# weiguangzhao/PBNet

Measured on AMD Instinct MI355X. Metric: scenes/sec fwd+cluster (ScanNet ~150k pts/scene), higher is better.
Workload: dtype bf16; 1 GPU; configs[1]: 1 scene, 161517 pts, 146038 voxels @2cm, 1 rotated copy, full PBNet.forward (MinkUNet34C + grouping + MinkUNet14A mask + MinkUNet34C score); scenes_in_flight_per_gpu=4, scene_seeds=2 (configs[1])

## Files before the change

pbnet_amd/csrc/cluster.hip:

```cpp
#include "pbn_common.h"

#pragma clang fp contract(off)

namespace pbn {
namespace {

constexpr int TPB = 256;
constexpr unsigned long long EMPTY_KEY = ~0ULL;
constexpr int CELL_BIAS = 32768;
constexpr float CELL_CLAMP = 32764.0f;
constexpr int CELL_R = 2;
constexpr int BIG = 0x7f7f7f7f;

__constant__ float c_mean_count[18] = {3917.0f, 12056.0f, 2303.0f, 8331.0f, 3948.0f, 3166.0f, 5629.0f, 11719.0f, 1003.0f,
                                       3317.0f, 4912.0f,  10221.0f, 3889.0f, 4136.0f, 2120.0f, 945.0f,  3967.0f, 2589.0f};

__device__ __forceinline__ float sqdist(float ax, float ay, float az, float bx, float by, float bz) {
    const float dx = __fsub_rn(ax, bx), dy = __fsub_rn(ay, by), dz = __fsub_rn(az, bz);
    const float a = __fmul_rn(dx, dx), b = __fmul_rn(dy, dy), c = __fmul_rn(dz, dz);
    return __fadd_rn(__fadd_rn(a, b), c);
}

__device__ __forceinline__ int cls_of(int sem) { return min(max(sem - 2, 0), 17); }

__device__ __forceinline__ int cell_coord(float v, float inv_cell) {
    float f = floorf(v * inv_cell);
    f = fminf(fmaxf(f, -CELL_CLAMP), CELL_CLAMP);
    return (int)f;
}

__device__ __forceinline__ unsigned long long pack_key(int seg, int cx, int cy, int cz) {
    return ((unsigned long long)(unsigned)seg << 48) | ((unsigned long long)(unsigned)(cx + CELL_BIAS) << 32) |
           ((unsigned long long)(unsigned)(cy + CELL_BIAS) << 16) | (unsigned long long)(unsigned)(cz + CELL_BIAS);
}

__device__ __forceinline__ int hash_lookup(const unsigned long long* __restrict__ hkeys, unsigned hmask,
                                           unsigned long long key) {
    unsigned h = hash64(key) & hmask;
    for (unsigned probes = 0; probes <= hmask; ++probes) {
        unsigned long long k = hkeys[h];
        if (k == key) return (int)h;
        if (k == EMPTY_KEY) return -1;
        h = (h + 1) & hmask;
    }
    return -1;
}

__global__ void k_seg_offsets(const int* __restrict__ seg_len, int n_seg, int n, int capacity, int* __restrict__ seg_off,
                              int* __restrict__ status) {
    const int lane = lane_id();
    int carry = 0;
    int bad = 0;
    for (int base = 0; base < n_seg; base += 64) {
        int i = base + lane;
        int v = (i < n_seg) ? seg_len[i] : 0;
        if (v < 0) bad = 1;
        int incl = v;
#pragma unroll
        for (int o = 1; o < 64; o <<= 1) {
            int t = __shfl_up(incl, o, 64);
            if (lane >= o) incl += t;
        }
        if (i < n_seg) seg_off[i] = carry + incl - v;
        carry += __shfl(incl, 63, 64);
    }
    bad = __any(bad);
    if (lane == 0) {
        seg_off[n_seg] = carry;
        if ((capacity ? carry > n : carry != n) || bad) atomicOr(status, 1);
    }
}

struct NRef {
    int cap;
    const int* dev;
    __device__ __forceinline__ int get() const { return dev ? min(cap, *dev) : cap; }
};

__device__ __forceinline__ int find_segment(const int* __restrict__ seg_off, int n_seg, int i) {
    int lo = 0, hi = n_seg;
    while (hi - lo > 1) {
        int mid = (lo + hi) >> 1;
        if (seg_off[mid] <= i) lo = mid; else hi = mid;
    }
    return lo;
}

__global__ __launch_bounds__(TPB) void k_cell_insert(const float* __restrict__ off_xyz, const int* __restrict__ sem,
                                                    const int* __restrict__ seg_off, int n_seg, NRef n_ref, float inv_cell,
                                                    unsigned long long* __restrict__ hkeys, int* __restrict__ hcount,
                                                    unsigned hmask, int* __restrict__ slot_of_pt,
                                                    int* __restrict__ seg_of_pt, int* __restrict__ status) {
    const int n = n_ref.get();
    const int i = blockIdx.x * TPB + threadIdx.x;
    if (i >= n) return;
    const int s = sem[i];
    if (s < 2 || s > 19) atomicOr(status, 2);
    const int seg = find_segment(seg_off, n_seg, i);
    seg_of_pt[i] = seg;
    const float x = off_xyz[3 * i + 0], y = off_xyz[3 * i + 1], z = off_xyz[3 * i + 2];
    const unsigned long long key = pack_key(seg, cell_coord(x, inv_cell), cell_coord(y, inv_cell), cell_coord(z, inv_cell));
    unsigned h = hash64(key) & hmask;
    bool placed = false;
    for (unsigned probes = 0; probes <= hmask; ++probes) {
        unsigned long long prev = atomicCAS(&hkeys[h], EMPTY_KEY, key);
        if (prev == EMPTY_KEY || prev == key) { placed = true; break; }
        h = (h + 1) & hmask;
    }
    if (!placed) { atomicOr(status, 4); h = 0; }
    atomicAdd(&hcount[h], 1);
    slot_of_pt[i] = (int)h;
}

__global__ __launch_bounds__(TPB) void k_cell_scatter(const float* __restrict__ off_xyz, NRef n_ref,
                                                     const int* __restrict__ slot_of_pt, const int* __restrict__ hstart,
                                                     int* __restrict__ hcursor, const int* __restrict__ seg_of_pt,
                                                     float4* __restrict__ spt, int* __restrict__ sseg,
                                                     int* __restrict__ sslot) {
    const int n = n_ref.get();
    const int i = blockIdx.x * TPB + threadIdx.x;
    if (i >= n) return;
    const int slot = slot_of_pt[i];
    const int pos = hstart[slot] + atomicAdd(&hcursor[slot], 1);
    spt[pos] = make_float4(off_xyz[3 * i + 0], off_xyz[3 * i + 1], off_xyz[3 * i + 2], __int_as_float(i));
    sseg[pos] = seg_of_pt[i];
    sslot[pos] = slot;
}

__device__ __forceinline__ bool cell_trusted(int cx, int cy, int cz) {
    const int lim = (int)CELL_CLAMP;
    return cx > -lim && cx < lim && cy > -lim && cy < lim && cz > -lim && cz < lim;
}

template <typename F>
__device__ __forceinline__ void for_each_neighbour_cell(float x, float y, float z, int seg, float inv_cell,
                                                        const unsigned long long* __restrict__ hkeys, unsigned hmask,
                                                        const int* __restrict__ hstart, const int* __restrict__ hcount,
                                                        int first, int stride, F&& f) {
    const int cx = cell_coord(x, inv_cell), cy = cell_coord(y, inv_cell), cz = cell_coord(z, inv_cell);
    constexpr int W = 2 * CELL_R + 1;
    for (int c = first; c < W * W * W; c += stride) {
        const int dz = c / (W * W) - CELL_R, dy = (c / W) % W - CELL_R, dx = c % W - CELL_R;
        const int slot = hash_lookup(hkeys, hmask, pack_key(seg, cx + dx, cy + dy, cz + dz));
        if (slot < 0) continue;
        const int beg = hstart[slot];
        f(beg, beg + hcount[slot], slot, cell_trusted(cx + dx, cy + dy, cz + dz), (dx | dy | dz) == 0);
    }
}

constexpr int NB_Q = 8;
__device__ __forceinline__ bool group_any(bool pred) {
    const unsigned long long m = __ballot(pred);
    return ((m >> (threadIdx.x & 63 & ~(NB_Q - 1))) & ((1ULL << NB_Q) - 1ULL)) != 0ULL;
}
template <typename F>
__device__ __forceinline__ void for_each_neighbour_cell_group(float x, float y, float z, int seg, float inv_cell,
                                                              const unsigned long long* __restrict__ hkeys, unsigned hmask,
                                                              const int* __restrict__ hstart,
                                                              const int* __restrict__ hcount, int q, F&& f) {
    const int cx = cell_coord(x, inv_cell), cy = cell_coord(y, inv_cell), cz = cell_coord(z, inv_cell);
    constexpr int W = 2 * CELL_R + 1;
    const int gbase = (threadIdx.x & 63) & ~(NB_Q - 1);
    for (int r = 0; r < W * W * W; r += NB_Q) {
        const int c = r + q;
        int slot = -1, beg = 0, end = 0;
        if (c < W * W * W) {
            const int dz = c / (W * W) - CELL_R, dy = (c / W) % W - CELL_R, dx = c % W - CELL_R;
            slot = hash_lookup(hkeys, hmask, pack_key(seg, cx + dx, cy + dy, cz + dz));
            if (slot >= 0) { beg = hstart[slot]; end = beg + hcount[slot]; }
        }
#pragma unroll
        for (int k = 0; k < NB_Q; ++k) {
            const int sk = __shfl(slot, gbase + k, 64);
            if (sk < 0) continue;
            const int bk = __shfl(beg, gbase + k, 64), ek = __shfl(end, gbase + k, 64);
            const int ck = r + k;
            const int dz = ck / (W * W) - CELL_R, dy = (ck / W) % W - CELL_R, dx = ck % W - CELL_R;
            f(bk, ek, sk, cell_trusted(cx + dx, cy + dy, cz + dz), (dx | dy | dz) == 0);
        }
    }
}
__device__ __forceinline__ int group_sum(int v) {
#pragma unroll
    for (int o = 1; o < NB_Q; o <<= 1) v += __shfl_xor(v, o, 64);
    return v;
}
__device__ __forceinline__ int group_max(int v) {
#pragma unroll
    for (int o = 1; o < NB_Q; o <<= 1) v = max(v, __shfl_xor(v, o, 64));
    return v;
}
__constant__ unsigned short c_nb_ring[125] = {
    146, 73,  74,  75,  81,  82,  83,  89,  90,  91,  137, 138, 139, 145, 147, 153, 154, 155, 201, 202, 203, 209, 210, 211, 217,
    218, 219, 0,   1,   2,   3,   4,   8,   9,   10,  11,  12,  16,  17,  18,  19,  20,  24,  25,  26,  27,  28,  32,  33,  34,
    35,  36,  64,  65,  66,  67,  68,  72,  76,  80,  84,  88,  92,  96,  97,  98,  99,  100, 128, 129, 130, 131, 132, 136, 140,
    144, 148, 152, 156, 160, 161, 162, 163, 164, 192, 193, 194, 195, 196, 200, 204, 208, 212, 216, 220, 224, 225, 226, 227, 228,
    256, 257, 258, 259, 260, 264, 265, 266, 267, 268, 272, 273, 274, 275, 276, 280, 281, 282, 283, 284, 288, 289, 290, 291, 292};

__global__ __launch_bounds__(TPB) void k_count(const float4* __restrict__ spt, const int* __restrict__ sseg,
                                              const int* __restrict__ sslot, NRef n_ref, float inv_cell, float r2,
                                              const unsigned long long* __restrict__ hkeys, unsigned hmask,
                                              const int* __restrict__ hstart, const int* __restrict__ hcount, int min_pts,
                                              int need_den, int* __restrict__ den) {
    __shared__ float4 s_cand[TPB / 64][64];
    const int n = n_ref.get();
    if (n <= 0) return;
    const long long t = (long long)blockIdx.x * TPB + threadIdx.x;
    if ((t - (threadIdx.x & 63)) / NB_Q >= n) return;
    int p = (int)(t / NB_Q);
    const int q = (int)(t % NB_Q);
    const bool live = p < n;
    if (!live) p = n - 1;
    const float4 me = spt[p];
    const int seg = sseg[p];
    const int lane = threadIdx.x & 63, wave = threadIdx.x >> 6;
    const int gbase = lane & ~(NB_Q - 1);
    float4* line = s_cand[wave];
    const int cx = cell_coord(me.x, inv_cell), cy = cell_coord(me.y, inv_cell), cz = cell_coord(me.z, inv_cell);
    const bool own_trusted = cell_trusted(cx, cy, cz);
    int cnt = (own_trusted && q == 0) ? hcount[sslot[p]] : 0;
    bool gdone = !live;
    if (!need_den) gdone = gdone || group_sum(cnt) > min_pts;
    bool wdone = __all(gdone);
    constexpr int NCELL = (2 * CELL_R + 1) * (2 * CELL_R + 1) * (2 * CELL_R + 1);
    for (int r = 0; r < NCELL && !wdone; r += NB_Q) {
        const int c = r + q;
        int slot = -1, beg = 0, end = 0;
        if (c < NCELL && !gdone && !(c == 0 && own_trusted)) {
            const int o = c_nb_ring[c];
            const int dx = (o & 7) - CELL_R, dy = ((o >> 3) & 7) - CELL_R, dz = (o >> 6) - CELL_R;
            slot = hash_lookup(hkeys, hmask, pack_key(seg, cx + dx, cy + dy, cz + dz));
            if (slot >= 0) { beg = hstart[slot]; end = beg + hcount[slot]; }
        }
        const bool same = beg == __shfl(beg, q, 64) && end == __shfl(end, q, 64);
        if (__all(same)) {
#pragma unroll 1
            for (int k = 0; k < NB_Q && !wdone; ++k) {
                const int bk = __shfl(beg, k, 64), ek = __shfl(end, k, 64);
                float4 nxt = make_float4(0.f, 0.f, 0.f, 0.f);
                if (bk + lane < ek) nxt = spt[bk + lane];
                for (int cb = bk; cb < ek; cb += 64) {
                    line[lane] = nxt;
                    if (cb + 64 + lane < ek) nxt = spt[cb + 64 + lane];
                    const int m = min(64, ek - cb);
#pragma unroll
                    for (int i = 0; i < 64 / NB_Q; ++i) {
                        const int idx = q + NB_Q * i;
                        if (idx < m) {
                            const float4 v = line[idx];
                            cnt += (sqdist(me.x, me.y, me.z, v.x, v.y, v.z) <= r2) ? 1 : 0;
                        }
                    }
                    if (!need_den) {
                        gdone = gdone || group_sum(cnt) > min_pts;
                        wdone = __all(gdone);
                        if (wdone) break;
                    }
                }
            }
        } else {
#pragma unroll
            for (int k = 0; k < NB_Q; ++k) {
                const int sk = __shfl(slot, gbase + k, 64);
                if (sk < 0 || gdone) continue;
                const int bk = __shfl(beg, gbase + k, 64), ek = __shfl(end, gbase + k, 64);
                int j = bk + q;
                for (; j + NB_Q < ek; j += 2 * NB_Q) {
                    const float4 q0 = spt[j], q1 = spt[j + NB_Q];
                    cnt += (sqdist(me.x, me.y, me.z, q0.x, q0.y, q0.z) <= r2) ? 1 : 0;
                    cnt += (sqdist(me.x, me.y, me.z, q1.x, q1.y, q1.z) <= r2) ? 1 : 0;
                }
                for (; j < ek; j += NB_Q) {
                    const float4 q0 = spt[j];
                    cnt += (sqdist(me.x, me.y, me.z, q0.x, q0.y, q0.z) <= r2) ? 1 : 0;
                }
                if (!need_den) gdone = group_sum(cnt) > min_pts;
            }
            wdone = __all(gdone);
        }
    }
    cnt = group_sum(cnt);
    if (live && q == 0) den[__float_as_int(me.w)] = need_den ? cnt - 1 : min(cnt - 1, min_pts);
}

__global__ __launch_bounds__(TPB) void k_tag_hp(float4* __restrict__ spt, NRef n_ref, const int* __restrict__ den, int min_pts,
                                               int* __restrict__ parent, int* __restrict__ lab,
                                               const int* __restrict__ sslot, int* __restrict__ cell_rep) {
    const int n = n_ref.get();
    const int p = blockIdx.x * TPB + threadIdx.x;
    if (p >= n) return;
    const int i = __float_as_int(spt[p].w);
    const int hp = den[i] >= min_pts;
    spt[p].w = __int_as_float(i | (hp ? (int)0x80000000 : 0));
    parent[i] = i;
    lab[i] = -1;
    if (hp) atomicMin(&cell_rep[sslot[p]], i);
}

__device__ __forceinline__ int uf_load(int* p) { return __hip_atomic_load(p, __ATOMIC_RELAXED, __HIP_MEMORY_SCOPE_AGENT); }

__device__ __forceinline__ int uf_find(int* __restrict__ parent, int x) {
    while (true) {
        const int p = uf_load(&parent[x]);
        if (p == x) return x;
        const int gp = uf_load(&parent[p]);
        if (gp == p) return p;
        atomicMin(&parent[x], gp);
        x = gp;
    }
}

__device__ __forceinline__ int uf_union(int* __restrict__ parent, int a, int b) {
    while (true) {
        a = uf_find(parent, a);
        b = uf_find(parent, b);
        if (a == b) return a;
        if (a < b) { const int t = a; a = b; b = t; }
        const int old = atomicMin(&parent[a], b);
        if (old == a) return b;
        a = old;
    }
}

template <int PASS>
__global__ __launch_bounds__(TPB) void k_union(const float4* __restrict__ spt, const int* __restrict__ sseg, NRef n_ref,
                                              float inv_cell, float r2, const unsigned long long* __restrict__ hkeys,
                                              unsigned hmask, const int* __restrict__ hstart,
                                              const int* __restrict__ hcount, int* parent,
                                              const int* __restrict__ cell_rep, const int* __restrict__ sslot,
                                              int* __restrict__ unres) {
    constexpr int pass = PASS;
    const int n = n_ref.get();
    const long long t = (long long)blockIdx.x * TPB + threadIdx.x;
    const int p = (int)(t / NB_Q), q = (int)(t % NB_Q);
    if (p >= n) return;
    const float4 me = spt[p];
    const int wi = __float_as_int(me.w);
    if (wi >= 0) return;
    const int i = wi & 0x7fffffff;
    const int my_slot = sslot[p];
    const bool own_trusted = cell_trusted(cell_coord(me.x, inv_cell), cell_coord(me.y, inv_cell), cell_coord(me.z, inv_cell));
    if (pass == 1 && own_trusted && !unres[my_slot]) return;
    const int my_rep = cell_rep[my_slot];
    bool unresolved = false;
    int ri = (pass == 0) ? i : parent[i];
    if (pass == 0 && own_trusted) {
        if (my_rep != i) {
            if (q == 0) uf_union(parent, i, my_rep);
            return;
        }
    }
    for_each_neighbour_cell(me.x, me.y, me.z, sseg[p], inv_cell, hkeys, hmask, hstart, hcount, q, NB_Q,
                            [&](int beg, int end, int slot, bool trusted, bool same) {
        const int rep = cell_rep[slot];
        if (rep == BIG) return;
        if (trusted) {
            if (same) return;
            if (rep == ri || parent[rep] == ri) return;
            ri = uf_find(parent, ri);
            if (uf_find(parent, rep) == ri) return;
            constexpr int WIT = PASS == 0 ? 8 : 1;
            for (int j = beg; j < end; j += WIT) {
                float4 c[WIT];
#pragma unroll
                for (int u = 0; u < WIT; ++u) c[u] = (j + u < end) ? spt[j + u] : make_float4(0.f, 0.f, 0.f, 0.f);
#pragma unroll
                for (int u = 0; u < WIT; ++u) {
                    if (__float_as_int(c[u].w) < 0 && sqdist(me.x, me.y, me.z, c[u].x, c[u].y, c[u].z) <= r2) {
                        ri = uf_union(parent, ri, __float_as_int(c[u].w) & 0x7fffffff);
                        return;
                    }
                }
            }
            unresolved = true;
            return;
        }
        unresolved = true;
        for (int j = beg; j < end; ++j) {
            const float4 q = spt[j];
            const int wj = __float_as_int(q.w);
            const int jj = wj & 0x7fffffff;
            if (wj < 0 && jj < i && sqdist(me.x, me.y, me.z, q.x, q.y, q.z) <= r2) {
                if (parent[jj] != ri) ri = uf_union(parent, ri, jj);
            }
        }
    });
    if (pass == 0 && own_trusted && unresolved) unres[my_slot] = 1;
}

__global__ __launch_bounds__(TPB) void k_compress(const float4* __restrict__ spt, NRef n_ref, int* parent) {
    const int n = n_ref.get();
    const int p = blockIdx.x * TPB + threadIdx.x;
    if (p >= n) return;
    const int wi = __float_as_int(spt[p].w);
    if (wi >= 0) return;
    const int i = wi & 0x7fffffff;
    const int r = uf_find(parent, i);
    if (r != i) atomicMin(&parent[i], r);
}

__global__ __launch_bounds__(TPB) void k_flatten(const float4* __restrict__ spt, NRef n_ref, int* __restrict__ parent,
                                                const int* __restrict__ sem, int general, int* __restrict__ semseed,
                                                int* __restrict__ lab) {
    const int n = n_ref.get();
    const int p = blockIdx.x * TPB + threadIdx.x;
    if (p >= n) return;
    const int wi = __float_as_int(spt[p].w);
    if (wi >= 0) return;
    const int i = wi & 0x7fffffff;
    const int r = uf_find(parent, i);
    lab[i] = r;
    if (general) atomicMin(&semseed[(size_t)cls_of(sem[i]) * n + r], i);
}

__global__ __launch_bounds__(TPB) void k_hp_seed_general(const float4* __restrict__ spt, NRef n_ref, const int* __restrict__ sem,
                                                        const int* __restrict__ semseed, int* __restrict__ lab) {
    const int n = n_ref.get();
    const int p = blockIdx.x * TPB + threadIdx.x;
    if (p >= n) return;
    const int wi = __float_as_int(spt[p].w);
    if (wi >= 0) return;
    const int i = wi & 0x7fffffff;
    lab[i] = semseed[(size_t)cls_of(sem[i]) * n + lab[i]];
}

__global__ __launch_bounds__(TPB) void k_border(const float4* __restrict__ spt, const int* __restrict__ sseg, NRef n_ref,
                                               float inv_cell, float r2, const unsigned long long* __restrict__ hkeys,
                                               unsigned hmask, const int* __restrict__ hstart,
                                               const int* __restrict__ hcount, const int* __restrict__ sem, int general,
                                               const int* __restrict__ semseed, const int* __restrict__ root,
                                               int* __restrict__ lab, const int* __restrict__ cell_rep) {
    const int n = n_ref.get();
    const long long t = (long long)blockIdx.x * TPB + threadIdx.x;
    if (n <= 0 || (t - (threadIdx.x & 63)) / NB_Q >= n) return;
    int p = (int)(t / NB_Q);
    const int q = (int)(t % NB_Q);
    const bool live = p < n;
    if (!live) p = n - 1;
    const float4 me = spt[p];
    const int wi = __float_as_int(me.w);
    if (wi < 0) return;
    const int i = wi;
    const int my_cls = cls_of(sem[i]);
    int best = -1;
    auto seed_of = [&](int hp_index) {
        int s = root[hp_index];
        if (general) {
            s = semseed[(size_t)my_cls * n + s];
            if (s == BIG) s = -1;
        }
        return s;
    };
    for_each_neighbour_cell_group(me.x, me.y, me.z, sseg[p], inv_cell, hkeys, hmask, hstart, hcount, q,
                                  [&](int beg, int end, int slot, bool trusted, bool same) {
        const int rep = cell_rep[slot];
        if (rep == BIG) return;
        if (trusted) {
            const int s = seed_of(rep);
            if (s <= best) return;
            if (same) { best = s; return; }
            for (int j0 = beg; j0 < end; j0 += NB_Q) {
                const int j = j0 + q;
                bool hit = false;
                if (j < end) {
                    const float4 c = spt[j];
                    hit = __float_as_int(c.w) < 0 && sqdist(me.x, me.y, me.z, c.x, c.y, c.z) <= r2;
                }
                if (group_any(hit)) { best = s; return; }
            }
            return;
        }
        for (int j0 = beg; j0 < end; j0 += NB_Q) {
            const int j = j0 + q;
            int cand = -1;
            if (j < end) {
                const float4 c = spt[j];
                const int wj = __float_as_int(c.w);
                if (wj < 0 && sqdist(me.x, me.y, me.z, c.x, c.y, c.z) <= r2) cand = seed_of(wj & 0x7fffffff);
            }
            best = max(best, group_max(cand));
        }
    });
    best = group_max(best);
    if (live && q == 0) lab[i] = best;
}

__global__ __launch_bounds__(TPB) void k_copy_i32(const int* __restrict__ src, int* __restrict__ dst, NRef n_ref) {
    const int n = n_ref.get();
    const int i = blockIdx.x * TPB + threadIdx.x;
    if (i < n) dst[i] = src[i];
}

__global__ __launch_bounds__(TPB) void k_sizes(const int* __restrict__ lab, NRef n_ref, int* __restrict__ size) {
    const int n = n_ref.get();
    const int i = blockIdx.x * TPB + threadIdx.x;
    int s = (i < n) ? lab[i] : -1;
    unsigned long long todo = __ballot(s >= 0);
    while (todo) {
        const int leader = __ffsll((long long)todo) - 1;
        const int ls = __shfl(s, leader, 64);
        const unsigned long long same = __ballot(s == ls);
        if (lane_id() == leader) atomicAdd(&size[ls], __popcll(same));
        todo &= ~same;
    }
}

__global__ __launch_bounds__(TPB) void k_keep(const int* __restrict__ lab, const int* __restrict__ size,
                                             const int* __restrict__ sem, NRef n_ref, float para_f, int* __restrict__ keep) {
    const int n = n_ref.get();
    const int i = blockIdx.x * TPB + threadIdx.x;
    if (i >= n) return;
    int k = 0;
    if (lab[i] == i) {
        const int cs = cls_of(sem[i]);
        const float thr = __fmul_rn(c_mean_count[cs], para_f);
        k = ((float)size[i] < thr) ? 0 : 1;
    }
    keep[i] = k;
}

__global__ __launch_bounds__(TPB) void k_relabel(const int* __restrict__ lab, const int* __restrict__ keep,
                                                const int* __restrict__ newid, const int* __restrict__ sem,
                                                const int* __restrict__ seg_of_pt, const float* __restrict__ org_xyz,
                                                NRef n_ref, int* __restrict__ lab2, int* __restrict__ cluster_id,
                                                int* __restrict__ clt_sem, int* __restrict__ clt_seg,
                                                int* __restrict__ last_assigned, int* __restrict__ fsize,
                                                int* __restrict__ noise_flag, float4* __restrict__ cand,
                                                const int* __restrict__ size) {
    const int n = n_ref.get();
    if (n <= 0) return;
    int i = blockIdx.x * TPB + threadIdx.x;
    if (i - (int)(threadIdx.x & 63) >= n) return;
    const bool live = i < n;
    if (!live) i = n - 1;
    const int s = lab[i];
    const int id = (s >= 0 && keep[s]) ? newid[s] : -1;
    if (live) {
        lab2[i] = id;
        cluster_id[i] = id;
        noise_flag[i] = id < 0;
    }
    if (keep[i]) {
        clt_sem[newid[i]] = sem[i];
        clt_seg[newid[i]] = seg_of_pt[i];
        fsize[newid[i]] = size[i];
    }
    {
        const int seg = seg_of_pt[i];
        const int cand_i = (id >= 0) ? i : -1;
        const int seg0 = __shfl(seg, 0, 64);
        if (__all(seg == seg0)) {
            int m = cand_i;
#pragma unroll
            for (int o = 32; o > 0; o >>= 1) m = max(m, __shfl_xor(m, o, 64));
            if (lane_id() == 0 && m >= 0) atomicMax(&last_assigned[seg0], m);
        } else if (cand_i >= 0) {
            atomicMax(&last_assigned[seg], cand_i);
        }
    }
    if (live)
        cand[i] = make_float4(org_xyz[3 * i + 0], org_xyz[3 * i + 1], org_xyz[3 * i + 2],
                              __int_as_float(id >= 0 ? ((seg_of_pt[i] << 8) | sem[i]) : -1));
}

__global__ void k_cluster_num(const int* __restrict__ newid, const int* __restrict__ seg_off, int n_seg, NRef n_ref,
                              const int* __restrict__ total, int* __restrict__ cluster_num,
                              const int* __restrict__ status, int* __restrict__ n_clusters) {
    const int n = n_ref.get();
    const int b = blockIdx.x * blockDim.x + threadIdx.x;
    if (b == 0) *n_clusters = (*status != 0) ? -1 : *total;
    if (b >= n_seg) return;
    const int lo = seg_off[b], hi = seg_off[b + 1];
    const int a = (lo < n) ? newid[lo] : *total;
    const int e = (hi < n) ? newid[hi] : *total;
    cluster_num[b] = e - a;
}

__global__ __launch_bounds__(TPB) void k_compact_noise(const int* __restrict__ noise_flag, const int* __restrict__ pos,
                                                      NRef n_ref, int* __restrict__ noise_list) {
    const int n = n_ref.get();
    const int i = blockIdx.x * TPB + threadIdx.x;
    if (i < n && noise_flag[i]) noise_list[pos[i]] = i;
}

__global__ __launch_bounds__(TPB) void k_noise_nn(const int* __restrict__ noise_list, const int* __restrict__ n_noise,
                                                 const float4* __restrict__ cand, const int* __restrict__ sem,
                                                 const int* __restrict__ seg_of_pt, const int* __restrict__ seg_off,
                                                 const int* __restrict__ lab2, const int* __restrict__ last_assigned,
                                                 int* __restrict__ cluster_id, int* __restrict__ fsize) {
    const int lane = lane_id();
    const int w = (int)(((long long)blockIdx.x * TPB + threadIdx.x) >> 6);
    if (w >= *n_noise) return;
    const int i = noise_list[w];
    const int seg = seg_of_pt[i];
    const int beg = seg_off[seg], end = seg_off[seg + 1];
    const float4 me = cand[i];
    const int key = (seg << 8) | sem[i];
    float best = __builtin_inff();
    int bi = -1;
    for (int j = beg + lane; j < end; j += 64) {
        const float4 q = cand[j];
        if (__float_as_int(q.w) == key) {
            const float d = sqdist(me.x, me.y, me.z, q.x, q.y, q.z);
            if (d <= best) { best = d; bi = j; }
        }
    }
#pragma unroll
    for (int o = 32; o > 0; o >>= 1) {
        const float ob = __shfl_xor(best, o, 64);
        const int oi = __shfl_xor(bi, o, 64);
        if (oi >= 0 && (bi < 0 || ob < best || (ob == best && oi > bi))) { best = ob; bi = oi; }
    }
    if (lane != 0) return;
    if (bi < 0) bi = last_assigned[seg];
    const int id = (bi >= 0) ? lab2[bi] : -1;
    cluster_id[i] = id;
    if (id >= 0) atomicAdd(&fsize[id], 1);
}

__device__ __forceinline__ float exact_quotient(float d, float n, float y) {
    const float q0 = __fmul_rn(d, y);
    const float r = __fmaf_rn(-q0, n, d);
    return __fmaf_rn(r, y, q0);
}

constexpr int CTR_TPB = 64;
constexpr int CTR_SUB = 4;
constexpr int CTR_CHUNK = CTR_TPB * CTR_SUB;
__global__ __launch_bounds__(CTR_TPB) void k_centers(const int* __restrict__ cluster_id, const float* __restrict__ off_xyz,
                                                    const int* __restrict__ clt_seg, const int* __restrict__ seg_off,
                                                    const int* __restrict__ n_clusters_total,
                                                    const int* __restrict__ member_start, int* __restrict__ member_idx,
                                                    float* __restrict__ centers) {
    __shared__ __attribute__((aligned(16))) float s_xyz[3][CTR_CHUNK + 32];
    __shared__ __attribute__((aligned(16))) float s_rcp[CTR_CHUNK + 32];
    const int lane = threadIdx.x;
    const int C = *n_clusters_total;
    for (int c = blockIdx.x; c < C; c += gridDim.x) {
        const int seg = clt_seg[c];
        const int beg = seg_off[seg], end = seg_off[seg + 1];
        int wpos = member_start[c];
        int N = 0;
        float m = 0.f;
        bool hit_n[CTR_SUB];
        float nx[CTR_SUB], ny[CTR_SUB], nz[CTR_SUB];
#pragma unroll
        for (int j = 0; j < CTR_SUB; ++j) {
            const int i = beg + j * CTR_TPB + lane;
            hit_n[j] = (i < end) && (cluster_id[i] == c);
            nx[j] = ny[j] = nz[j] = 0.f;
            if (hit_n[j]) { nx[j] = off_xyz[3 * i + 0]; ny[j] = off_xyz[3 * i + 1]; nz[j] = off_xyz[3 * i + 2]; }
        }
        for (int base = beg; base < end; base += CTR_CHUNK) {
            bool hit[CTR_SUB];
            float px[CTR_SUB], py[CTR_SUB], pz[CTR_SUB];
#pragma unroll
            for (int j = 0; j < CTR_SUB; ++j) { hit[j] = hit_n[j]; px[j] = nx[j]; py[j] = ny[j]; pz[j] = nz[j]; }
#pragma unroll
            for (int j = 0; j < CTR_SUB; ++j) {
                const int i = base + CTR_CHUNK + j * CTR_TPB + lane;
                hit_n[j] = (i < end) && (cluster_id[i] == c);
                if (hit_n[j]) { nx[j] = off_xyz[3 * i + 0]; ny[j] = off_xyz[3 * i + 1]; nz[j] = off_xyz[3 * i + 2]; }
            }
            int cnt = 0;
            bool ok = true;
#pragma unroll
            for (int j = 0; j < CTR_SUB; ++j) {
                const unsigned long long mask = __ballot(hit[j]);
                const int rank = cnt + __popcll(mask & ((1ULL << lane) - 1ULL));
                cnt += __popcll(mask);
                const float ax = fabsf(px[j]), ay = fabsf(py[j]), az = fabsf(pz[j]);
                ok = ok && (!hit[j] || ((ax == 0.f || (ax >= 1e-20f && ax <= 1e20f)) && (ay == 0.f || (ay >= 1e-20f && ay <= 1e20f)) &&
                                        (az == 0.f || (az >= 1e-20f && az <= 1e20f))));
                if (hit[j]) {
                    s_xyz[0][rank] = px[j]; s_xyz[1][rank] = py[j]; s_xyz[2][rank] = pz[j];
                    if (member_idx) member_idx[wpos + rank] = base + j * CTR_TPB + lane;
                }
            }
            if (cnt == 0) continue;
            const bool fast = __all(ok);
#pragma unroll
            for (int j = 0; j < CTR_SUB; ++j)
                if (j * CTR_TPB < cnt) s_rcp[j * CTR_TPB + lane] = __fdiv_rn(1.0f, (float)(N + 1 + j * CTR_TPB + lane));
            wpos += cnt;
            __syncthreads();
            if (lane < 3) {
                const float* v = s_xyz[lane];
                if (fast) {
                    float4 va[4], ya[4], vb[4], yb[4];
                    auto load16 = [&](float4 (&vv)[4], float4 (&yy)[4], int k) {
#pragma unroll
                        for (int q = 0; q < 4; ++q) {
                            vv[q] = *reinterpret_cast<const float4*>(v + k + 4 * q);
                            yy[q] = *reinterpret_cast<const float4*>(s_rcp + k + 4 * q);
                        }
                    };
                    auto chain16 = [&](const float4 (&vv)[4], const float4 (&yy)[4], int k) {
                        const float n0 = (float)(N + k + 1);
                        const int left = cnt - k;
                        if (left >= 16) {
#pragma unroll
                            for (int q = 0; q < 4; ++q) {
                                m = __fadd_rn(m, exact_quotient(__fsub_rn(vv[q].x, m), n0 + (float)(4 * q + 0), yy[q].x));
                                m = __fadd_rn(m, exact_quotient(__fsub_rn(vv[q].y, m), n0 + (float)(4 * q + 1), yy[q].y));
                                m = __fadd_rn(m, exact_quotient(__fsub_rn(vv[q].z, m), n0 + (float)(4 * q + 2), yy[q].z));
                                m = __fadd_rn(m, exact_quotient(__fsub_rn(vv[q].w, m), n0 + (float)(4 * q + 3), yy[q].w));
                            }
                        } else {
                            for (int j = 0; j < left; ++j)
                                m = __fadd_rn(m, exact_quotient(__fsub_rn(v[k + j], m), n0 + (float)j, s_rcp[k + j]));
                        }
                    };
                    load16(va, ya, 0);
                    for (int k = 0; k < cnt; k += 32) {
                        load16(vb, yb, k + 16);
                        chain16(va, ya, k);
                        if (k + 16 < cnt) {
                            load16(va, ya, k + 32);
                            chain16(vb, yb, k + 16);
                        }
                    }
                } else {
                    for (int k = 0; k < cnt; ++k) m = __fadd_rn(m, __fdiv_rn(__fsub_rn(v[k], m), (float)(N + k + 1)));
                }
            }
            N += cnt;
            __syncthreads();
        }
        if (lane < 3) centers[3 * c + lane] = m;
    }
}

__global__ void k_member_tail(int* __restrict__ member_start, const int* __restrict__ total_assigned, int n,
                              const int* __restrict__ n_clusters) {
    if (threadIdx.x == 0 && blockIdx.x == 0) member_start[n] = *total_assigned;
    (void)n_clusters;
}

struct Workspace {
    int *seg_off, *seg_of_pt, *slot_of_pt, *hcount, *hstart, *hcursor, *unres, *sseg, *sslot, *cell_rep, *parent, *lab, *root, *semseed, *size,
        *keep, *newid, *lab2, *clt_seg, *last_assigned, *fsize, *noise_flag, *noise_pos, *noise_list, *scan_tmp,
        *scalars, *mstart_tmp;
    unsigned long long* scan_state[4];
    unsigned long long* hkeys;
    float4 *spt, *cand;
    unsigned hcap;
    size_t zero_end, ff_end, big_end;
};

unsigned hash_capacity(int n) {
    unsigned c = 1024;
    while (c < 2u * (unsigned)n) c <<= 1;
    return c;
}

size_t carve(Carver& cv, Workspace& w, int n, int n_seg, int general) {
    const size_t N = (size_t)(n > 0 ? n : 1);
    w.hcap = hash_capacity(n);
    w.scalars = cv.take<int>(64);
    for (int j = 0; j < 4; ++j)
        w.scan_state[j] = cv.take<unsigned long long>(scan_chained_state_words((long long)(w.hcap > N ? w.hcap : N)));
    w.hcount = cv.take<int>(w.hcap);
    w.hcursor = cv.take<int>(w.hcap);
    w.unres = cv.take<int>(w.hcap);
    w.size = cv.take<int>(N);
    w.fsize = cv.take<int>(N);
    w.zero_end = cv.off;
    w.hkeys = cv.take<unsigned long long>(w.hcap);
    w.last_assigned = cv.take<int>((size_t)n_seg + 1);
    w.ff_end = cv.off;
    w.cell_rep = cv.take<int>(w.hcap);
    w.semseed = cv.take<int>(general ? 18 * N : 1);
    w.big_end = cv.off;
    w.hstart = cv.take<int>(w.hcap);
    w.spt = cv.take<float4>(N);
    w.cand = cv.take<float4>(N);
    w.seg_off = cv.take<int>((size_t)n_seg + 1);
    w.seg_of_pt = cv.take<int>(N);
    w.slot_of_pt = cv.take<int>(N);
    w.sseg = cv.take<int>(N);
    w.sslot = cv.take<int>(N);
    w.parent = cv.take<int>(N);
    w.lab = cv.take<int>(N);
    w.root = cv.take<int>(N);
    w.keep = cv.take<int>(N);
    w.newid = cv.take<int>(N);
    w.lab2 = cv.take<int>(N);
    w.clt_seg = cv.take<int>(N);
    w.noise_flag = cv.take<int>(N);
    w.noise_pos = cv.take<int>(N);
    w.noise_list = cv.take<int>(N);
    w.mstart_tmp = cv.take<int>(N + 1);
    w.scan_tmp = cv.take<int>(scan_tmp_ints((long long)(w.hcap > N ? w.hcap : N)));
    return align_up(cv.off, 256);
}

}
}

using namespace pbn;

extern "C" size_t pbn_cluster_workspace_bytes(int n_points, int n_segments, int general_sem) {
    if (n_points < 0 || n_segments < 0) return 0;
    Carver cv(nullptr, 0);
    Workspace w;
    return carve(cv, w, n_points, n_segments, general_sem);
}

extern "C" int pbn_binary_cluster(const float* off_xyz, const float* org_xyz, const int32_t* sem,
                                  const int32_t* seg_len, int n, int n_seg, float radius, int min_pts, float para_f,
                                  int nv_flag, int flags, int32_t* cluster_id, int32_t* cluster_num, int32_t* den,
                                  float* centers, int32_t* clt_sem, int32_t* n_clusters, int32_t* member_start,
                                  int32_t* member_idx, void* workspace, size_t workspace_bytes, pbn_stream_t stream_) {
    hipStream_t stream = (hipStream_t)stream_;
    const int general = flags & 1;
    const int capacity = (flags >> 1) & 1;
    const int need_den = !((flags >> 2) & 1);
    if (n < 0 || n_seg < 0 || n_seg > 65535 || !(radius > 0.0f) || !n_clusters || (n_seg > 0 && !cluster_num))
        return PBN_ERR_ARG;
    if ((member_start == nullptr) != (member_idx == nullptr)) return PBN_ERR_ARG;
    if (n > 0 && (!off_xyz || !org_xyz || !sem || !seg_len || !cluster_id || !den || !centers || !clt_sem || !workspace))
        return PBN_ERR_ARG;
    if (n == 0 || n_seg == 0) {
        if (n_seg > 0) { const int frc_ = fill_bytes(cluster_num, 0, sizeof(int) * (size_t)n_seg, stream); if (frc_ != PBN_OK) return frc_; }
        { const int frc_ = fill_bytes(n_clusters, 0, sizeof(int), stream); if (frc_ != PBN_OK) return frc_; }
        if (member_start) { const int frc_ = fill_bytes(member_start, 0, sizeof(int) * ((size_t)n + 1), stream); if (frc_ != PBN_OK) return frc_; }
        return PBN_OK;
    }
    Carver cv(workspace, workspace_bytes);
    Workspace w;
    carve(cv, w, n, n_seg, general);
    if (!cv.ok) return PBN_ERR_WORKSPACE;

    const float cell = radius * 0.5625f;
    const float inv_cell = 1.0f / cell;
    const float r2 = radius * radius;
    const unsigned hmask = w.hcap - 1;
    const int nb = cdiv(n, TPB);
    const NRef nr{n, capacity ? w.seg_off + n_seg : nullptr};
    int* status = w.scalars + 0;
    int* total_kept = w.scalars + 1;
    int* n_noise = w.scalars + 2;
    int* total_assigned = w.scalars + 3;

    {
        char* base = (char*)workspace;
        char* z0 = (char*)w.scalars;
        char* f0 = (char*)w.hkeys;
        char* b0 = (char*)w.cell_rep;
        FillRange fr[7] = {{cluster_num, sizeof(int) * (size_t)n_seg, 0}, {n_clusters, sizeof(int), 0},
                           {z0, (size_t)(base + w.zero_end - z0), 0}, {f0, (size_t)(base + w.ff_end - f0), 0xff},
                           {b0, (size_t)(base + w.big_end - b0), 0x7f}, {nullptr, 0, 0}, {nullptr, 0, 0}};
        if (capacity) {
            fr[5] = FillRange{w.keep, sizeof(int) * (size_t)n, 0};
            fr[6] = FillRange{w.noise_flag, sizeof(int) * (size_t)n, 0};
        }
        const int frc = fill_ranges(fr, 7, stream);
        if (frc != PBN_OK) return frc;
    }

    hipLaunchKernelGGL(k_seg_offsets, dim3(1), dim3(64), 0, stream, seg_len, n_seg, n, capacity, w.seg_off, status);
    hipLaunchKernelGGL(k_cell_insert, dim3(nb), dim3(TPB), 0, stream, off_xyz, sem, w.seg_off, n_seg, nr, inv_cell,
                       w.hkeys, w.hcount, hmask, w.slot_of_pt, w.seg_of_pt, status);
    int rc = scan_exclusive_i32_chained(w.hcount, w.hstart, (int)w.hcap, w.scan_state[0], nullptr, status, stream);
    if (rc != PBN_OK) return rc;
    hipLaunchKernelGGL(k_cell_scatter, dim3(nb), dim3(TPB), 0, stream, off_xyz, nr, w.slot_of_pt, w.hstart, w.hcursor,
                       w.seg_of_pt, w.spt, w.sseg, w.sslot);
    hipLaunchKernelGGL(k_count, dim3(cdiv((long long)n * NB_Q, TPB)), dim3(TPB), 0, stream, w.spt, w.sseg, w.sslot, nr, inv_cell, r2,
                       w.hkeys, hmask, w.hstart, w.hcount, min_pts, need_den, den);
    hipLaunchKernelGGL(k_tag_hp, dim3(nb), dim3(TPB), 0, stream, w.spt, nr, den, min_pts, w.parent, w.lab, w.sslot, w.cell_rep);
    const dim3 nbq(cdiv((long long)n * NB_Q, TPB));
    hipLaunchKernelGGL(k_union<0>, nbq, dim3(TPB), 0, stream, w.spt, w.sseg, nr, inv_cell, r2, w.hkeys, hmask,
                       w.hstart, w.hcount, w.parent, w.cell_rep, w.sslot, w.unres);
    hipLaunchKernelGGL(k_compress, dim3(nb), dim3(TPB), 0, stream, w.spt, nr, w.parent);
    hipLaunchKernelGGL(k_union<1>, nbq, dim3(TPB), 0, stream, w.spt, w.sseg, nr, inv_cell, r2, w.hkeys, hmask,
                       w.hstart, w.hcount, w.parent, w.cell_rep, w.sslot, w.unres);
    hipLaunchKernelGGL(k_flatten, dim3(nb), dim3(TPB), 0, stream, w.spt, nr, w.parent, sem, general, w.semseed, w.lab);
    hipLaunchKernelGGL(k_copy_i32, dim3(nb), dim3(TPB), 0, stream, w.lab, w.root, nr);
    if (general)
        hipLaunchKernelGGL(k_hp_seed_general, dim3(nb), dim3(TPB), 0, stream, w.spt, nr, sem, w.semseed, w.lab);
    hipLaunchKernelGGL(k_border, nbq, dim3(TPB), 0, stream, w.spt, w.sseg, nr, inv_cell, r2, w.hkeys, hmask,
                       w.hstart, w.hcount, sem, general, w.semseed, w.root, w.lab, w.cell_rep);
    hipLaunchKernelGGL(k_sizes, dim3(nb), dim3(TPB), 0, stream, w.lab, nr, w.size);
    hipLaunchKernelGGL(k_keep, dim3(nb), dim3(TPB), 0, stream, w.lab, w.size, sem, nr, para_f, w.keep);
    rc = scan_exclusive_i32_chained(w.keep, w.newid, n, w.scan_state[1], total_kept, status, stream);
    if (rc != PBN_OK) return rc;
    hipLaunchKernelGGL(k_relabel, dim3(nb), dim3(TPB), 0, stream, w.lab, w.keep, w.newid, sem, w.seg_of_pt, org_xyz, nr,
                       w.lab2, cluster_id, clt_sem, w.clt_seg, w.last_assigned, w.fsize, w.noise_flag, w.cand, w.size);
    hipLaunchKernelGGL(k_cluster_num, dim3(cdiv(n_seg, 64)), dim3(64), 0, stream, w.newid, w.seg_off, n_seg, nr,
                       total_kept, cluster_num, status, n_clusters);
    if (nv_flag) {
        rc = scan_exclusive_i32_chained(w.noise_flag, w.noise_pos, n, w.scan_state[2], n_noise, status, stream);
        if (rc != PBN_OK) return rc;
        hipLaunchKernelGGL(k_compact_noise, dim3(nb), dim3(TPB), 0, stream, w.noise_flag, w.noise_pos, nr, w.noise_list);
        hipLaunchKernelGGL(k_noise_nn, dim3(cdiv((long long)n * 64, TPB)), dim3(TPB), 0, stream, w.noise_list, n_noise, w.cand, sem, w.seg_of_pt,
                           w.seg_off, w.lab2, w.last_assigned, cluster_id, w.fsize);
    }
    int* mstart = member_start ? member_start : w.mstart_tmp;
    rc = scan_exclusive_i32_chained(w.fsize, mstart, n, w.scan_state[3], total_assigned, status, stream);
    if (rc != PBN_OK) return rc;
    hipLaunchKernelGGL(k_member_tail, dim3(1), dim3(64), 0, stream, mstart, total_assigned, n, total_kept);
    const int center_blocks = 2048;
    hipLaunchKernelGGL(k_centers, dim3(center_blocks), dim3(CTR_TPB), 0, stream, cluster_id, off_xyz, w.clt_seg, w.seg_off,
                       total_kept, mstart, member_idx, centers);
    PBN_LAUNCH_CHECK();
    return PBN_OK;
}
```

Before: 376.6 scenes/s.

## Split cluster centers into parallel member gather and deep-pipelined sequential mean

Member gathering and center computation are split into two kernels. A 1024-thread k_members kernel counts per-wave hits, writes member indices and SoA coordinates to global memory, precomputes reciprocals, and records a per-cluster fast-path flag. k_centers then runs the exact sequential running-mean chain from global memory with a six-deep load pipeline. The aim is to take the gather off the serial critical path and hide load latency, at the cost of an extra kernel launch, extra global traffic and more registers. Optional timing stamps are added behind a compile flag.

```diff
diff --git a/pbnet_amd/csrc/cluster.hip b/pbnet_amd/csrc/cluster.hip
--- a/pbnet_amd/csrc/cluster.hip
+++ b/pbnet_amd/csrc/cluster.hip
@@ -624,110 +624,169 @@
     return __fmaf_rn(r, y, q0);
 }
 
+constexpr int MB_TPB = 1024;
+constexpr int MB_WAVES = MB_TPB / 64;
+constexpr int MB_COUNT_SLICES = 8;
+constexpr int MB_WRITE_SLICES = 4;
 constexpr int CTR_TPB = 64;
-constexpr int CTR_SUB = 4;
-constexpr int CTR_CHUNK = CTR_TPB * CTR_SUB;
-__global__ __launch_bounds__(CTR_TPB) void k_centers(const int* __restrict__ cluster_id, const float* __restrict__ off_xyz,
-                                                    const int* __restrict__ clt_seg, const int* __restrict__ seg_off,
-                                                    const int* __restrict__ n_clusters_total,
-                                                    const int* __restrict__ member_start, int* __restrict__ member_idx,
-                                                    float* __restrict__ centers) {
-    __shared__ __attribute__((aligned(16))) float s_xyz[3][CTR_CHUNK + 32];
-    __shared__ __attribute__((aligned(16))) float s_rcp[CTR_CHUNK + 32];
-    const int lane = threadIdx.x;
+constexpr int CTR_DEPTH = 6;
+constexpr int CTR_PAD = 16 * (CTR_DEPTH + 1);
+
+#ifdef PBN_CENTERS_TIMING
+constexpr int CTR_STAMPED = 64;
+__device__ unsigned long long g_centers_timing[CTR_STAMPED * 8];
+#define CTR_STAMP(I) do { if (c < CTR_STAMPED && threadIdx.x == 0) g_centers_timing[c * 8 + (I)] = wall_clock64(); } while (0)
+#else
+#define CTR_STAMP(I)
+#endif
+
+__global__ __launch_bounds__(MB_TPB) void k_members(const int* __restrict__ cluster_id, const float* __restrict__ off_xyz,
+                                                   const int* __restrict__ clt_seg, const int* __restrict__ seg_off,
+                                                   const int* __restrict__ n_clusters_total,
+                                                   const int* __restrict__ member_start, NRef n_ref,
+                                                   int* __restrict__ member_idx, float* __restrict__ mxyz, size_t plane,
+                                                   float* __restrict__ rcp, int* __restrict__ clt_fast) {
+    __shared__ int s_cnt[MB_WAVES];
+    __shared__ int s_ok[MB_WAVES];
+    const int lane = lane_id();
+    const int wave = threadIdx.x >> 6;
+    const int n = n_ref.get();
+    for (long long j = (long long)blockIdx.x * MB_TPB + threadIdx.x; j < n; j += (long long)gridDim.x * MB_TPB)
+        rcp[j] = __fdiv_rn(1.0f, (float)(j + 1));
     const int C = *n_clusters_total;
     for (int c = blockIdx.x; c < C; c += gridDim.x) {
         const int seg = clt_seg[c];
         const int beg = seg_off[seg], end = seg_off[seg + 1];
+        CTR_STAMP(1);
+        const int per = (int)((((long long)(end - beg) + MB_TPB - 1) / MB_TPB) * 64);
+        const long long wb_ll = (long long)beg + (long long)wave * per;
+        const int wb = (int)(wb_ll < end ? wb_ll : end);
+        const int we = (int)(wb_ll + per < end ? wb_ll + per : end);
+        int mine = 0;
+        for (int base = wb; base < we; base += 64 * MB_COUNT_SLICES) {
+#pragma unroll
+            for (int j = 0; j < MB_COUNT_SLICES; ++j) {
+                const int i = base + j * 64 + lane;
+                mine += (i < we && cluster_id[i] == c) ? 1 : 0;
+            }
+        }
+#pragma unroll
+        for (int o = 32; o > 0; o >>= 1) mine += __shfl_xor(mine, o, 64);
+        if (lane == 0) s_cnt[wave] = mine;
+        __syncthreads();
         int wpos = member_start[c];
-        int N = 0;
+        for (int w = 0; w < wave; ++w) wpos += s_cnt[w];
+        CTR_STAMP(2);
+        bool ok = true;
+        for (int base = wb; base < we; base += 64 * MB_WRITE_SLICES) {
+            bool hit[MB_WRITE_SLICES];
+            float px[MB_WRITE_SLICES], py[MB_WRITE_SLICES], pz[MB_WRITE_SLICES];
+#pragma unroll
+            for (int j = 0; j < MB_WRITE_SLICES; ++j) {
+                const int i = base + j * 64 + lane;
+                hit[j] = i < we && cluster_id[i] == c;
+                px[j] = py[j] = pz[j] = 0.f;
+                if (hit[j]) { px[j] = off_xyz[3 * (size_t)i + 0]; py[j] = off_xyz[3 * (size_t)i + 1]; pz[j] = off_xyz[3 * (size_t)i + 2]; }
+            }
+#pragma unroll
+            for (int j = 0; j < MB_WRITE_SLICES; ++j) {
+                const unsigned long long mask = __ballot(hit[j]);
+                const int pos = wpos + __popcll(mask & ((1ULL << lane) - 1ULL));
+                wpos += __popcll(mask);
+                const float ax = fabsf(px[j]), ay = fabsf(py[j]), az = fabsf(pz[j]);
+                ok = ok && ((ax == 0.f || (ax >= 1e-20f && ax <= 1e20f)) && (ay == 0.f || (ay >= 1e-20f && ay <= 1e20f)) &&
+                            (az == 0.f || (az >= 1e-20f && az <= 1e20f)));
+                if (hit[j]) {
+                    if (member_idx) member_idx[pos] = base + j * 64 + lane;
+                    mxyz[pos] = px[j]; mxyz[plane + pos] = py[j]; mxyz[2 * plane + pos] = pz[j];
+                }
+            }
+        }
+        const int wave_ok = __all(ok);
+        if (lane == 0) s_ok[wave] = wave_ok;
+        __syncthreads();
+        if (threadIdx.x == 0) {
+            int all_ok = 1;
+            for (int w = 0; w < MB_WAVES; ++w) all_ok &= s_ok[w];
+            clt_fast[c] = all_ok;
+        }
+        CTR_STAMP(3);
+    }
+}
+
+struct __attribute__((packed, aligned(4))) Float4U { float x, y, z, w; };
+
+__global__ __launch_bounds__(CTR_TPB) void k_centers(const int* __restrict__ n_clusters_total, const int* __restrict__ member_start,
+                                                    const float* __restrict__ mxyz, size_t plane, const float* __restrict__ rcp,
+                                                    const int* __restrict__ clt_fast, float* __restrict__ centers) {
+    const int lane = threadIdx.x;
+    if (lane >= 3) return;
+    const int C = *n_clusters_total;
+    for (int c = blockIdx.x; c < C; c += gridDim.x) {
+        const int ms = member_start[c];
+        const int cnt = member_start[c + 1] - ms;
+#ifdef PBN_CENTERS_TIMING
+        if (c < CTR_STAMPED && lane == 0) g_centers_timing[c * 8] = (unsigned long long)cnt;
+#endif
+        CTR_STAMP(4);
+        const float* v = mxyz + (size_t)lane * plane + ms;
+        int vz = 0;
+        asm volatile("" : "+v"(vz));
+        const float* y = rcp + vz;
         float m = 0.f;
-        bool hit_n[CTR_SUB];
-        float nx[CTR_SUB], ny[CTR_SUB], nz[CTR_SUB];
-#pragma unroll
-        for (int j = 0; j < CTR_SUB; ++j) {
-            const int i = beg + j * CTR_TPB + lane;
-            hit_n[j] = (i < end) && (cluster_id[i] == c);
-            nx[j] = ny[j] = nz[j] = 0.f;
-            if (hit_n[j]) { nx[j] = off_xyz[3 * i + 0]; ny[j] = off_xyz[3 * i + 1]; nz[j] = off_xyz[3 * i + 2]; }
-        }
-        for (int base = beg; base < end; base += CTR_CHUNK) {
-            bool hit[CTR_SUB];
-            float px[CTR_SUB], py[CTR_SUB], pz[CTR_SUB];
-#pragma unroll
-            for (int j = 0; j < CTR_SUB; ++j) { hit[j] = hit_n[j]; px[j] = nx[j]; py[j] = ny[j]; pz[j] = nz[j]; }
-#pragma unroll
-            for (int j = 0; j < CTR_SUB; ++j) {
-                const int i = base + CTR_CHUNK + j * CTR_TPB + lane;
-                hit_n[j] = (i < end) && (cluster_id[i] == c);
-                if (hit_n[j]) { nx[j] = off_xyz[3 * i + 0]; ny[j] = off_xyz[3 * i + 1]; nz[j] = off_xyz[3 * i + 2]; }
-            }
-            int cnt = 0;
-            bool ok = true;
-#pragma unroll
-            for (int j = 0; j < CTR_SUB; ++j) {
-                const unsigned long long mask = __ballot(hit[j]);
-                const int rank = cnt + __popcll(mask & ((1ULL << lane) - 1ULL));
-                cnt += __popcll(mask);
-                const float ax = fabsf(px[j]), ay = fabsf(py[j]), az = fabsf(pz[j]);
-                ok = ok && (!hit[j] || ((ax == 0.f || (ax >= 1e-20f && ax <= 1e20f)) && (ay == 0.f || (ay >= 1e-20f && ay <= 1e20f)) &&
-                                        (az == 0.f || (az >= 1e-20f && az <= 1e20f))));
-                if (hit[j]) {
-                    s_xyz[0][rank] = px[j]; s_xyz[1][rank] = py[j]; s_xyz[2][rank] = pz[j];
-                    if (member_idx) member_idx[wpos + rank] = base + j * CTR_TPB + lane;
+        if (clt_fast[c]) {
+            Float4U vv[CTR_DEPTH][4];
+            float4 yy[CTR_DEPTH][4];
+            auto load16 = [&](int slot, int k) {
+#pragma unroll
+                for (int q = 0; q < 4; ++q) {
+                    vv[slot][q] = *reinterpret_cast<const Float4U*>(v + k + 4 * q);
+                    yy[slot][q] = *reinterpret_cast<const float4*>(y + k + 4 * q);
                 }
-            }
-            if (cnt == 0) continue;
-            const bool fast = __all(ok);
-#pragma unroll
-            for (int j = 0; j < CTR_SUB; ++j)
-                if (j * CTR_TPB < cnt) s_rcp[j * CTR_TPB + lane] = __fdiv_rn(1.0f, (float)(N + 1 + j * CTR_TPB + lane));
-            wpos += cnt;
-            __syncthreads();
-            if (lane < 3) {
-                const float* v = s_xyz[lane];
-                if (fast) {
-                    float4 va[4], ya[4], vb[4], yb[4];
-                    auto load16 = [&](float4 (&vv)[4], float4 (&yy)[4], int k) {
-#pragma unroll
-                        for (int q = 0; q < 4; ++q) {
-                            vv[q] = *reinterpret_cast<const float4*>(v + k + 4 * q);
-                            yy[q] = *reinterpret_cast<const float4*>(s_rcp + k + 4 * q);
-                        }
-                    };
-                    auto chain16 = [&](const float4 (&vv)[4], const float4 (&yy)[4], int k) {
-                        const float n0 = (float)(N + k + 1);
-                        const int left = cnt - k;
-                        if (left >= 16) {
-#pragma unroll
-                            for (int q = 0; q < 4; ++q) {
-                                m = __fadd_rn(m, exact_quotient(__fsub_rn(vv[q].x, m), n0 + (float)(4 * q + 0), yy[q].x));
-                                m = __fadd_rn(m, exact_quotient(__fsub_rn(vv[q].y, m), n0 + (float)(4 * q + 1), yy[q].y));
-                                m = __fadd_rn(m, exact_quotient(__fsub_rn(vv[q].z, m), n0 + (float)(4 * q + 2), yy[q].z));
-                                m = __fadd_rn(m, exact_quotient(__fsub_rn(vv[q].w, m), n0 + (float)(4 * q + 3), yy[q].w));
-                            }
-                        } else {
-                            for (int j = 0; j < left; ++j)
-                                m = __fadd_rn(m, exact_quotient(__fsub_rn(v[k + j], m), n0 + (float)j, s_rcp[k + j]));
-                        }
-                    };
-                    load16(va, ya, 0);
-                    for (int k = 0; k < cnt; k += 32) {
-                        load16(vb, yb, k + 16);
-                        chain16(va, ya, k);
-                        if (k + 16 < cnt) {
-                            load16(va, ya, k + 32);
-                            chain16(vb, yb, k + 16);
-                        }
+            };
+            auto chain16 = [&](int slot, int k) {
+                const float n0 = (float)(k + 1);
+#pragma unroll
+                for (int q = 0; q < 4; ++q) {
+                    m = __fadd_rn(m, exact_quotient(__fsub_rn(vv[slot][q].x, m), n0 + (float)(4 * q + 0), yy[slot][q].x));
+                    m = __fadd_rn(m, exact_quotient(__fsub_rn(vv[slot][q].y, m), n0 + (float)(4 * q + 1), yy[slot][q].y));
+                    m = __fadd_rn(m, exact_quotient(__fsub_rn(vv[slot][q].z, m), n0 + (float)(4 * q + 2), yy[slot][q].z));
+                    m = __fadd_rn(m, exact_quotient(__fsub_rn(vv[slot][q].w, m), n0 + (float)(4 * q + 3), yy[slot][q].w));
+                }
+            };
+#pragma unroll
+            for (int s = 0; s < CTR_DEPTH; ++s) load16(s, 16 * s);
+            int k = 0;
+            for (; k + 16 * CTR_DEPTH <= cnt; k += 16 * CTR_DEPTH) {
+#pragma unroll
+                for (int s = 0; s < CTR_DEPTH; ++s) {
+                    chain16(s, k + 16 * s);
+                    __builtin_amdgcn_sched_barrier(0);
+                    load16(s, k + 16 * s + 16 * CTR_DEPTH);
+                    __builtin_amdgcn_sched_barrier(0);
+                }
+            }
+#pragma unroll
+            for (int s = 0; s < CTR_DEPTH; ++s) {
+                const int left = cnt - (k + 16 * s);
+                if (left >= 16) {
+                    chain16(s, k + 16 * s);
+                } else if (left > 0) {
+                    const float n0 = (float)(k + 16 * s + 1);
+#pragma unroll
+                    for (int q = 0; q < 4; ++q) {
+                        if (4 * q + 0 < left) m = __fadd_rn(m, exact_quotient(__fsub_rn(vv[s][q].x, m), n0 + (float)(4 * q + 0), yy[s][q].x));
+                        if (4 * q + 1 < left) m = __fadd_rn(m, exact_quotient(__fsub_rn(vv[s][q].y, m), n0 + (float)(4 * q + 1), yy[s][q].y));
+                        if (4 * q + 2 < left) m = __fadd_rn(m, exact_quotient(__fsub_rn(vv[s][q].z, m), n0 + (float)(4 * q + 2), yy[s][q].z));
+                        if (4 * q + 3 < left) m = __fadd_rn(m, exact_quotient(__fsub_rn(vv[s][q].w, m), n0 + (float)(4 * q + 3), yy[s][q].w));
                     }
-                } else {
-                    for (int k = 0; k < cnt; ++k) m = __fadd_rn(m, __fdiv_rn(__fsub_rn(v[k], m), (float)(N + k + 1)));
                 }
             }
-            N += cnt;
-            __syncthreads();
-        }
-        if (lane < 3) centers[3 * c + lane] = m;
+        } else {
+            for (int k = 0; k < cnt; ++k) m = __fadd_rn(m, __fdiv_rn(__fsub_rn(v[k], m), (float)(k + 1)));
+        }
+        CTR_STAMP(5);
+        centers[3 * c + lane] = m;
     }
 }
 
@@ -740,7 +799,9 @@
 struct Workspace {
     int *seg_off, *seg_of_pt, *slot_of_pt, *hcount, *hstart, *hcursor, *unres, *sseg, *sslot, *cell_rep, *parent, *lab, *root, *semseed, *size,
         *keep, *newid, *lab2, *clt_seg, *last_assigned, *fsize, *noise_flag, *noise_pos, *noise_list, *scan_tmp,
-        *scalars, *mstart_tmp;
+        *scalars, *mstart_tmp, *clt_fast;
+    float *mxyz, *rcp;
+    size_t mplane;
     unsigned long long* scan_state[4];
     unsigned long long* hkeys;
     float4 *spt, *cand;
@@ -791,6 +852,10 @@
     w.noise_pos = cv.take<int>(N);
     w.noise_list = cv.take<int>(N);
     w.mstart_tmp = cv.take<int>(N + 1);
+    w.clt_fast = cv.take<int>(N);
+    w.mplane = align_up(N + CTR_PAD, 4);
+    w.mxyz = cv.take<float>(3 * w.mplane);
+    w.rcp = cv.take<float>(w.mplane);
     w.scan_tmp = cv.take<int>(scan_tmp_ints((long long)(w.hcap > N ? w.hcap : N)));
     return align_up(cv.off, 256);
 }
@@ -901,8 +966,18 @@
     if (rc != PBN_OK) return rc;
     hipLaunchKernelGGL(k_member_tail, dim3(1), dim3(64), 0, stream, mstart, total_assigned, n, total_kept);
     const int center_blocks = 2048;
-    hipLaunchKernelGGL(k_centers, dim3(center_blocks), dim3(CTR_TPB), 0, stream, cluster_id, off_xyz, w.clt_seg, w.seg_off,
-                       total_kept, mstart, member_idx, centers);
+    hipLaunchKernelGGL(k_members, dim3(center_blocks), dim3(MB_TPB), 0, stream, cluster_id, off_xyz, w.clt_seg, w.seg_off,
+                       total_kept, mstart, nr, member_idx, w.mxyz, w.mplane, w.rcp, w.clt_fast);
+    hipLaunchKernelGGL(k_centers, dim3(center_blocks), dim3(CTR_TPB), 0, stream, total_kept, mstart, w.mxyz, w.mplane, w.rcp,
+                       w.clt_fast, centers);
     PBN_LAUNCH_CHECK();
     return PBN_OK;
 }
+
+#ifdef PBN_CENTERS_TIMING
+extern "C" int pbn_centers_timing_read(unsigned long long* host) {
+    PBN_HIP_CHECK(hipDeviceSynchronize());
+    PBN_HIP_CHECK(hipMemcpyFromSymbol(host, HIP_SYMBOL(pbn::g_centers_timing), sizeof(unsigned long long) * (pbn::CTR_STAMPED * 8)));
+    return PBN_OK;
+}
+#endif
```

Result: faster. 383.7 scenes/s, median of 6 (+1.9%).
